# taichi-dev/taichi-nerfs

Hardware: AMD Instinct MI355X
Metric: training rays/sec (higher is better)
Workload: dtype f32-table+f16-mlp

## Files before the change

### taichi-nerfs_amd/csrc/march.hip

```cpp
#include "ngp_device.h"
#include "march_common.h"
#include <stdlib.h>

namespace ngp {

__global__ void __launch_bounds__(256) ray_aabb_kernel(const float* __restrict__ rays_o, const float* __restrict__ rays_d,
                                                        float scale, int n, float2* __restrict__ hits_t) {
    int r = blockIdx.x * blockDim.x + threadIdx.x;
    if (r >= n) return;
    float o[3], d_inv[3];
#pragma unroll
    for (int k = 0; k < 3; ++k) { o[k] = rays_o[3 * r + k]; d_inv[k] = 1.0f / rays_d[3 * r + k]; }
    hits_t[r] = ray_aabb_slab(o, d_inv, scale);
}

constexpr int MARCH_GROUP = 32;

template <bool CONST_DT, int G, bool CASC1>
__device__ __forceinline__ int march_rays_of_wave(const float* __restrict__ rays_o, const float* __restrict__ rays_d,
                                                  const float2* __restrict__ hits_t, const uint8_t* __restrict__ bits,
                                                  const float* __restrict__ noise, const MarchParams& p, int max_samples, int n_rays,
                                                  const uint32_t* __restrict__ coarse_s, bool use_coarse, float2* __restrict__ stage,
                                                  unsigned long long* __restrict__ chain, int first_ray, float o[3], float d[3]) {
    const int lane = threadIdx.x & 63;
    const int grp = lane / G, sub = lane % G;
    const int r = first_ray + grp;
    const bool has_ray = r < n_rays;
    const int rr = has_ray ? r : 0;
    float d_inv[3];
#pragma unroll
    for (int k = 0; k < 3; ++k) { o[k] = rays_o[3 * rr + k]; d[k] = rays_d[3 * rr + k]; d_inv[k] = 1.0f / d[k]; }
    float2 h;
    if (hits_t) h = hits_t[rr];
    else h = ray_aabb_slab(o, d_inv, p.scale);
    float t1 = h.x;
    const float t2 = h.y;
    const float dt_c = calc_dt(0.0f, p.esf, p.dt_min, p.dt_max);
    if (t1 >= 0.0f) t1 += calc_dt(t1, p.esf, p.dt_min, p.dt_max) * (p.rng ? rng_uniform(p.rng_seed, (unsigned int)rr) : noise[rr]);
    float t = t1;
    int n = 0;
    float t_target = -INFINITY;
    float2* row = stage + (size_t)rr * (size_t)max_samples;
    bool live = has_ray && (0.0f <= t) && (t < t2) && (n < max_samples);
    while (__any(live)) {
        float tu = t, t_last = t, tt = t;
        if (CONST_DT) {
#pragma unroll
            for (int k = 0; k < G; ++k) {
                tu = (k == sub) ? tt : tu;
                t_last = tt;
                tt += dt_c;
            }
        } else {
            for (int k = 0; k < G; ++k) {
                if (k == sub) tu = tt;
                t_last = tt;
                tt += calc_dt(tt, p.esf, p.dt_min, p.dt_max);
            }
        }
        const float t_next_batch = tt;
        const float dtu = CONST_DT ? dt_c : calc_dt(tu, p.esf, p.dt_min, p.dt_max);
        const float t_after = tu + dtu;
        CellProbe c;
        probe_cell<CASC1>(p, o, d, tu, dtu, c);
        bool occ = live;
        if (use_coarse && occ) { const uint32_t cb = c.idx >> 9; occ = (coarse_s[cb >> 5] >> (cb & 31u)) & 1u; }
        if (occ) occ = (bits[c.idx >> 3] >> (c.idx & 7u)) & 1u;
        const float targ = skip_target(p, d, d_inv, tu, c);
        const unsigned long long interesting = __ballot(live && (occ || targ > t_after));
        const unsigned long long gmask = (G == 64) ? ~0ull : (((1ull << (G & 63)) - 1ull) << ((grp * G) & 63));
        const bool need = (interesting & gmask) != 0ull;
        if (!need) {
            if (live) {
                if (!(t_last < t2)) live = false;
                if (!(t_target > t_last)) t_target = -INFINITY;
            }
        }
        if (interesting != 0ull) {
            const unsigned long long GM = (G == 64) ? ~0ull : ((1ull << (G & 63)) - 1ull);
            const int gbase = grp * G;
            const int gsh = gbase & 63;
            const bool act = live && need;
            const int nv = __popcll((__ballot(tu < t2) >> gsh) & GM);
            const int e0 = __popcll((__ballot(tu < t_target) >> gsh) & GM);
            const unsigned long long occm = (__ballot(occ) >> gsh) & GM;
            int c = 0;
#pragma unroll
            for (int s = G / 2; s >= 1; s >>= 1) {
                const float tv = __shfl(tu, gbase + c + s - 1);
                if (tv < targ) c += s;
            }
            if (__shfl(tu, gbase + G - 1) < targ) c = G;
            int j = occ ? sub + 1 : max(sub + 1, c);
            if (sub == 0) chain[grp] = (e0 < G) ? (1ull << e0) : 0ull;
            bool on_chain = sub == e0;
#pragma unroll
            for (int k = 1; k < G; k <<= 1) {
                wave_sync_lds();
                if (on_chain && j < G) atomicOr(&chain[grp], 1ull << j);
                wave_sync_lds();
                on_chain = (chain[grp] >> sub) & 1ull;
                if (2 * k < G) {
                    const int jj = __shfl(j, gbase + min(j, G - 1));
                    j = (j >= G) ? G : jj;
                }
            }
            const unsigned long long inside = (nv >= 64) ? ~0ull : ((1ull << nv) - 1ull);
            const unsigned long long X = act ? (chain[grp] & inside) : 0ull;
            const unsigned long long E = X & occm;
            const int cnt = __popcll(E), cap = max_samples - n;
            const int rank = __popcll(E & ((1ull << sub) - 1ull));
            if (((E >> sub) & 1ull) && rank < cap) row[n + rank] = make_float2(tu, dtu);
            const int last = X ? 63 - __clzll(X) : 0;
            const float targ_last = __shfl(targ, gbase + last);
            if (act) {
                if (X) t_target = ((occm >> last) & 1ull) ? -INFINITY : targ_last;
                const bool full = cnt >= cap;
                n = full ? max_samples : n + cnt;
                live = !full && nv == G;
            }
            wave_sync_lds();
        }
        t = t_next_batch;
    }
    return n;
}


template <bool CONST_DT, int G, bool CASC1>
__global__ void __launch_bounds__(64) march_count_kernel(const float* __restrict__ rays_o, const float* __restrict__ rays_d,
                                                         const float2* __restrict__ hits_t,
                                                         const uint8_t* __restrict__ bits, const float* __restrict__ noise,
                                                         MarchParams p, int max_samples, int n_rays,
                                                         const uint32_t* __restrict__ coarse ,
                                                         float2* __restrict__ stage, int32_t* __restrict__ counts) {
    constexpr int GROUPS = 64 / G;
    __shared__ unsigned long long chain[GROUPS];
    __shared__ uint32_t coarse_s[MARCH_MAX_COARSE_WORDS];
    const bool use_coarse = load_coarse(p, coarse, coarse_s);
    float o[3], d[3];
    const int n = march_rays_of_wave<CONST_DT, G, CASC1>(rays_o, rays_d, hits_t, bits, noise, p, max_samples, n_rays, coarse_s, use_coarse,
                                                         stage, chain, blockIdx.x * GROUPS, o, d);
    const int r = blockIdx.x * GROUPS + (int)threadIdx.x / G;
    if (r < n_rays && threadIdx.x % G == 0) counts[r] = n;
}

#ifdef NGP_MARCH_DIAG
__device__ unsigned long long ngp_march_dbg[4 * 8192];
#endif

template <bool CONST_DT, int G, bool CASC1, int WAVES>
__global__ void __launch_bounds__(64 * WAVES) march_fused_kernel(const float* __restrict__ rays_o, const float* __restrict__ rays_d,
                                                           const float2* __restrict__ hits_t, const uint8_t* __restrict__ bits,
                                                           const float* __restrict__ noise, MarchParams p, int max_samples, int n_rays,
                                                           const uint32_t* __restrict__ coarse, float2* __restrict__ stage,
                                                           int32_t* __restrict__ ctr, int32_t* __restrict__ rays_a,
                                                           int32_t* __restrict__ total, float* __restrict__ xyzs,
                                                           float* __restrict__ dirs, float* __restrict__ deltas, float* __restrict__ ts) {
    constexpr int GROUPS = 64 / G, RPB = WAVES * GROUPS;
    static_assert(RPB <= 64, "wave 0 scans the block's ray counts with one wave scan");
    __shared__ unsigned long long chain[WAVES][GROUPS];
    __shared__ uint32_t coarse_s[MARCH_MAX_COARSE_WORDS];
    __shared__ int s_off[RPB];
    const bool use_coarse = load_coarse(p, coarse, coarse_s);
    const int wv = threadIdx.x >> 6, lane = threadIdx.x & 63, grp = lane / G, sub = lane % G;
    const int first = blockIdx.x * RPB + wv * GROUPS, r = first + grp;
    float o[3], d[3];
#ifdef NGP_MARCH_DIAG
    const unsigned long long t_w0 = wall_clock64();
#endif
    const int n = march_rays_of_wave<CONST_DT, G, CASC1>(rays_o, rays_d, hits_t, bits, noise, p, max_samples, n_rays, coarse_s, use_coarse,
                                                         stage, chain[wv], first, o, d);
#ifdef NGP_MARCH_DIAG
    if (lane == 0 && blockIdx.x * WAVES + wv < 8192) {
        unsigned long long* q = ngp_march_dbg + 4 * (blockIdx.x * WAVES + wv);
        q[0] = t_w0; q[1] = wall_clock64(); q[3] = (unsigned long long)n;
    }
#endif
    const bool has_ray = r < n_rays;
    if (sub == 0) s_off[wv * GROUPS + grp] = has_ray ? n : 0;
    __threadfence_block();
    __syncthreads();
    if (wv == 0) {
        const int c = lane < RPB ? s_off[lane] : 0;
        const int inc = wave_scan_add_i(c, lane);
        int base = 0;
        if (lane == NGP_WAVE - 1) base = atomicAdd(&ctr[0], inc);
        base = __shfl(base, NGP_WAVE - 1, NGP_WAVE);
        if (lane < RPB) s_off[lane] = base + inc - c;
    }
    __syncthreads();
    if (has_ray) {
        const int start = s_off[wv * GROUPS + grp];
        if (sub == 0) { rays_a[3 * r] = r; rays_a[3 * r + 1] = start; rays_a[3 * r + 2] = n; }
        const float2* row = stage + (size_t)r * (size_t)max_samples;
        for (int k = sub; k < n; k += G) {
            const float2 s = row[k];
            const size_t g = (size_t)start + k;
            if (p.capacity > 0 && (long long)g >= p.capacity) break;
#pragma unroll
            for (int a = 0; a < 3; ++a) {
                xyzs[3 * g + a] = o[a] + s.x * d[a];
                dirs[3 * g + a] = d[a];
            }
            ts[g] = s.x;
            deltas[g] = s.y;
        }
    }
#ifdef NGP_MARCH_DIAG
    if (lane == 0 && blockIdx.x * WAVES + wv < 8192) ngp_march_dbg[4 * (blockIdx.x * WAVES + wv) + 2] = wall_clock64();
#endif
    if (threadIdx.x == 0) {
        if (atomicAdd(&ctr[1], 1) == (int)gridDim.x - 1) {
            total[0] = atomicExch(&ctr[0], 0);
            atomicExch(&ctr[1], 0);
        }
    }
}

__global__ void __launch_bounds__(256) bitfield_coarsen_kernel(const uint4* __restrict__ bits16, int n_coarse,
                                                               uint32_t* __restrict__ coarse) {
    const int w = blockIdx.x * blockDim.x + threadIdx.x;
    bool any = false;
    if (w < n_coarse) {
#pragma unroll
        for (int k = 0; k < 4; ++k) { const uint4 v = bits16[4 * (size_t)w + k]; any |= (v.x | v.y | v.z | v.w) != 0u; }
    }
    const unsigned long long m = __ballot(any);
    const int lane = threadIdx.x & 63;
    if (lane == 0 && w < n_coarse) coarse[w >> 5] = (uint32_t)m;
    if (lane == 32 && w < n_coarse) coarse[w >> 5] = (uint32_t)(m >> 32);
}

__global__ void __launch_bounds__(1024) march_scan_kernel(const int32_t* __restrict__ counts, int n_rays,
                                                          int32_t* __restrict__ rays_a, int32_t* __restrict__ total) {
    __shared__ int wave_tot[16];
    const int tid = threadIdx.x, lane = tid & 63, wv = tid >> 6;
    const int per = (n_rays + 1023) >> 10;
    const int lo = min(tid * per, n_rays), hi = min(lo + per, n_rays);
    int sum = 0;
    for (int i = lo; i < hi; ++i) sum += counts[i];
    const int inc = wave_scan_add_i(sum, lane);
    if (lane == 63) wave_tot[wv] = inc;
    __syncthreads();
    int woff = 0;
#pragma unroll
    for (int w = 0; w < 16; ++w) woff += (w < wv) ? wave_tot[w] : 0;
    int run = woff + inc - sum;
    for (int i = lo; i < hi; ++i) {
        const int c = counts[i];
        rays_a[3 * i] = i; rays_a[3 * i + 1] = run; rays_a[3 * i + 2] = c;
        run += c;
    }
    if (tid == 1023) total[0] = woff + inc;
}

__global__ void __launch_bounds__(1024) live_compact_kernel(const int32_t* __restrict__ rays_a, const int32_t* __restrict__ vr_per_ray,
                                                            int n_rays, int32_t* __restrict__ live_off, int32_t* __restrict__ live_idx,
                                                            int32_t* __restrict__ live_total) {
    __shared__ int wave_tot[16];
    const int tid = threadIdx.x, lane = tid & 63, wv = tid >> 6;
    const int per = (n_rays + 1023) >> 10;
    const int lo = min(tid * per, n_rays), hi = min(lo + per, n_rays);
    int sum = 0;
    for (int i = lo; i < hi; ++i) sum += vr_per_ray[i];
    const int inc = wave_scan_add_i(sum, lane);
    if (lane == 63) wave_tot[wv] = inc;
    __syncthreads();
    int woff = 0;
#pragma unroll
    for (int w = 0; w < 16; ++w) woff += (w < wv) ? wave_tot[w] : 0;
    int run = woff + inc - sum;
    for (int i = lo; i < hi; ++i) { live_off[i] = run; run += vr_per_ray[i]; }
    if (blockIdx.x == 0 && tid == 1023) live_total[0] = woff + inc;
    __threadfence_block();
    __syncthreads();
    const int share = (n_rays + (int)gridDim.x - 1) / (int)gridDim.x;
    const int n0 = blockIdx.x * share, n1 = min(n0 + share, n_rays);
    for (int n = n0 + wv; n < n1; n += 16) {
        const int ray = rays_a[3 * n], start = rays_a[3 * n + 1];
        const int cnt = vr_per_ray[ray], base = live_off[ray];
        for (int k = lane; k < cnt; k += NGP_WAVE) live_idx[base + k] = start + k;
    }
}

__global__ void __launch_bounds__(256) march_write_kernel(const float* __restrict__ rays_o, const float* __restrict__ rays_d,
                                                          const int32_t* __restrict__ rays_a, const float2* __restrict__ stage,
                                                          int max_samples, int n_rays, float* __restrict__ xyzs,
                                                          float* __restrict__ dirs, float* __restrict__ deltas,
                                                          float* __restrict__ ts) {
    int r = blockIdx.x * (blockDim.x >> 6) + (threadIdx.x >> 6);
    if (r >= n_rays) return;
    const int lane = lane_id();
    const int start = rays_a[3 * r + 1], cnt = rays_a[3 * r + 2];
    if (cnt == 0) return;
    float o[3], d[3];
#pragma unroll
    for (int k = 0; k < 3; ++k) { o[k] = rays_o[3 * r + k]; d[k] = rays_d[3 * r + k]; }
    const float2* row = stage + (size_t)r * (size_t)max_samples;
    for (int k = lane; k < cnt; k += NGP_WAVE) {
        float2 s = row[k];
        size_t g = (size_t)start + k;
#pragma unroll
        for (int a = 0; a < 3; ++a) {
            xyzs[3 * g + a] = o[a] + s.x * d[a];
            dirs[3 * g + a] = d[a];
        }
        ts[g] = s.x;
        deltas[g] = s.y;
    }
}

__global__ void __launch_bounds__(64) march_test_kernel(const float* __restrict__ rays_o, const float* __restrict__ rays_d,
                                                        float* __restrict__ hits_t, const int64_t* __restrict__ alive,
                                                        const uint8_t* __restrict__ bits, MarchParams p, int max_samples,
                                                        int n_alive, int64_t* __restrict__ ray_indices,
                                                        uint8_t* __restrict__ valid_mask, float* __restrict__ deltas,
                                                        float* __restrict__ ts, int32_t* __restrict__ samples_counter) {
    int n = blockIdx.x * blockDim.x + threadIdx.x;
    if (n >= n_alive) return;
    const int64_t r = alive[n];
    float o[3], d[3], d_inv[3];
#pragma unroll
    for (int k = 0; k < 3; ++k) { o[k] = rays_o[3 * r + k]; d[k] = rays_d[3 * r + k]; d_inv[k] = 1.0f / d[k]; }
    float t = hits_t[2 * r];
    const float t2 = hits_t[2 * r + 1];
    int s = 0;
    const size_t base = (size_t)n * (size_t)max_samples;
    float t_target = -INFINITY;
    float t_resume = t;
    bool wrote = false;
    bool live = (0.0f < t) && (t < t2) && (s < max_samples);
    while (live) {
        float tb[ORBIT_BATCH], dtb[ORBIT_BATCH];
        uint8_t ob[ORBIT_BATCH];
        uint32_t ib[ORBIT_BATCH];
        float tt = t;
#pragma unroll
        for (int u = 0; u < ORBIT_BATCH; ++u) {
            float dt = calc_dt(tt, p.esf, p.dt_min, p.dt_max);
            CellProbe c;
            probe_cell<false>(p, o, d, tt, dt, c);
            tb[u] = tt; dtb[u] = dt; ib[u] = c.idx;
            ob[u] = bits[c.idx >> 3];
            tt += dt;
        }
#pragma unroll
        for (int u = 0; u < ORBIT_BATCH; ++u) {
            if (!live) break;
            float tu = tb[u];
            if (!(tu < t2)) { live = false; break; }
            if (tu < t_target) continue;
            if (ob[u] & (1u << (ib[u] & 7u))) {
                size_t i = base + s;
                ray_indices[i] = r; valid_mask[i] = 1; ts[i] = tu; deltas[i] = dtb[u];
                t_resume = tu + dtb[u]; wrote = true;
                s += 1;
                t_target = -INFINITY;
                if (s >= max_samples) live = false;
            } else {
                CellProbe c;
                probe_cell<false>(p, o, d, tu, dtb[u], c);
                t_target = skip_target(p, d, d_inv, tu, c);
            }
        }
        t = tt;
    }
    if (wrote) hits_t[2 * r] = t_resume;
    samples_counter[n] = s;
}

}

using namespace ngp;

extern "C" {

int ngp_ray_aabb(const float* rays_o, const float* rays_d, float scale, int n_rays, float* hits_t, void* stream) {
    if (n_rays <= 0) return 0;
    hipLaunchKernelGGL(ray_aabb_kernel, dim3((n_rays + 255) / 256), dim3(256), 0, (hipStream_t)stream, rays_o, rays_d, scale,
                       n_rays, (float2*)hits_t);
    NGP_LAUNCH_CHECK();
    return 0;
}

int ngp_bitfield_coarsen(const uint8_t* density_bitfield, int cascades, int grid_size, uint32_t* coarse, void* stream) {
    const long long cells = (long long)cascades * grid_size * grid_size * grid_size;
    if (cells <= 0 || cells % 512 != 0) return -1;
    const int n_coarse = (int)(cells / 512);
    if (n_coarse % 32 != 0) return -1;
    hipLaunchKernelGGL(bitfield_coarsen_kernel, dim3((n_coarse + 255) / 256), dim3(256), 0, (hipStream_t)stream,
                       (const uint4*)density_bitfield, n_coarse, coarse);
    NGP_LAUNCH_CHECK();
    return 0;
}

int ngp_march_train_count(const float* rays_o, const float* rays_d, const float* hits_t, const uint8_t* density_bitfield,
                          const float* noise, int cascades, int grid_size, float scale, float exp_step_factor,
                          int max_samples, int n_rays, float* stage, int32_t* counts, void* stream) {
    return ngp_march_train_count_ex(rays_o, rays_d, hits_t, density_bitfield, nullptr, noise, cascades, grid_size, scale,
                                    exp_step_factor, max_samples, n_rays, stage, counts, stream);
}

int ngp_march_train_count_ex(const float* rays_o, const float* rays_d, const float* hits_t, const uint8_t* density_bitfield,
                             const uint32_t* coarse, const float* noise, int cascades, int grid_size, float scale,
                             float exp_step_factor, int max_samples, int n_rays, float* stage, int32_t* counts, void* stream) {
    if (n_rays <= 0) return 0;
    MarchParams p = make_march_params(cascades, grid_size, scale, exp_step_factor);
    const char* ge = ngp_experiment("march_group");
    const int group = ge ? atoi(ge) : MARCH_GROUP;
    hipStream_t s = (hipStream_t)stream;
#define NGP_LAUNCH_MARCH(CD, GG, C1)                                                                                           \
    hipLaunchKernelGGL((march_count_kernel<CD, GG, C1>), dim3((n_rays + 64 / GG - 1) / (64 / GG)), dim3(64), 0, s, rays_o,     \
                       rays_d, (const float2*)hits_t, density_bitfield, noise, p, max_samples, n_rays, coarse, (float2*)stage, \
                       counts)
    const bool cd = exp_step_factor == 0.0f, c1 = cascades == 1;
    if (group == 64) {
        if (cd && c1) NGP_LAUNCH_MARCH(true, 64, true); else if (cd) NGP_LAUNCH_MARCH(true, 64, false);
        else if (c1) NGP_LAUNCH_MARCH(false, 64, true); else NGP_LAUNCH_MARCH(false, 64, false);
    } else if (group == 16) {
        if (cd && c1) NGP_LAUNCH_MARCH(true, 16, true); else if (cd) NGP_LAUNCH_MARCH(true, 16, false);
        else if (c1) NGP_LAUNCH_MARCH(false, 16, true); else NGP_LAUNCH_MARCH(false, 16, false);
    } else {
        if (cd && c1) NGP_LAUNCH_MARCH(true, 32, true); else if (cd) NGP_LAUNCH_MARCH(true, 32, false);
        else if (c1) NGP_LAUNCH_MARCH(false, 32, true); else NGP_LAUNCH_MARCH(false, 32, false);
    }
#undef NGP_LAUNCH_MARCH
    NGP_LAUNCH_CHECK();
    return 0;
}

static int march_train_fused(const float* rays_o, const float* rays_d, const float* hits_t, const uint8_t* density_bitfield,
                             const uint32_t* coarse, const float* noise, bool rng, unsigned long long seed, int cascades, int grid_size,
                             float scale, float exp_step_factor, int max_samples, int n_rays, float* stage, int32_t* ctr, int32_t* rays_a,
                             int32_t* total, float* xyzs, float* dirs, float* deltas, float* ts, void* stream, long long capacity = 0,
                             int block_waves = 16, int lds_pad = 0) {
    if (n_rays <= 0) return 0;
    if (!ctr || !rays_a || !total || (!rng && !noise) || capacity < 0) return -1;
    if ((block_waves != 16 && block_waves != 8 && block_waves != 4) || lds_pad < 0 || lds_pad > 150 * 1024) return -1;
    MarchParams p = make_march_params(cascades, grid_size, scale, exp_step_factor);
    p.rng = rng ? 1 : 0; p.rng_seed = seed; p.capacity = capacity;
    hipStream_t s = (hipStream_t)stream;
    const int rpb = block_waves * (64 / MARCH_GROUP);
#define NGP_LAUNCH_MARCH_W(CD, C1, W)                                                                                               \
    hipLaunchKernelGGL((march_fused_kernel<CD, MARCH_GROUP, C1, W>), dim3((n_rays + rpb - 1) / rpb), dim3(64 * W), (size_t)lds_pad, s,   \
                       rays_o, rays_d, (const float2*)hits_t, density_bitfield, noise, p, max_samples, n_rays, coarse, (float2*)stage,  \
                       ctr, rays_a, total, xyzs, dirs, deltas, ts)
#define NGP_LAUNCH_MARCH(CD, C1)                                                                                                    \
    do { if (block_waves == 16) NGP_LAUNCH_MARCH_W(CD, C1, 16); else if (block_waves == 8) NGP_LAUNCH_MARCH_W(CD, C1, 8);           \
         else NGP_LAUNCH_MARCH_W(CD, C1, 4); } while (0)
    const bool cd = exp_step_factor == 0.0f, c1 = cascades == 1;
    if (cd && c1) NGP_LAUNCH_MARCH(true, true); else if (cd) NGP_LAUNCH_MARCH(true, false);
    else if (c1) NGP_LAUNCH_MARCH(false, true); else NGP_LAUNCH_MARCH(false, false);
#undef NGP_LAUNCH_MARCH
#undef NGP_LAUNCH_MARCH_W
    NGP_LAUNCH_CHECK();
    return 0;
}

int ngp_march_train_fused(const float* rays_o, const float* rays_d, const float* hits_t, const uint8_t* density_bitfield,
                          const uint32_t* coarse, const float* noise, int cascades, int grid_size, float scale, float exp_step_factor,
                          int max_samples, int n_rays, float* stage, int32_t* ctr, int32_t* rays_a, int32_t* total, float* xyzs,
                          float* dirs, float* deltas, float* ts, void* stream) {
    return march_train_fused(rays_o, rays_d, hits_t, density_bitfield, coarse, noise, false, 0ull, cascades, grid_size, scale,
                             exp_step_factor, max_samples, n_rays, stage, ctr, rays_a, total, xyzs, dirs, deltas, ts, stream);
}

int ngp_march_train_fused_cap(const float* rays_o, const float* rays_d, const float* hits_t, const uint8_t* density_bitfield,
                              const uint32_t* coarse, const float* noise, int cascades, int grid_size, float scale,
                              float exp_step_factor, int max_samples, int n_rays, long long capacity, float* stage, int32_t* ctr,
                              int32_t* rays_a, int32_t* total, float* xyzs, float* dirs, float* deltas, float* ts, void* stream) {
    return march_train_fused(rays_o, rays_d, hits_t, density_bitfield, coarse, noise, false, 0ull, cascades, grid_size, scale,
                             exp_step_factor, max_samples, n_rays, stage, ctr, rays_a, total, xyzs, dirs, deltas, ts, stream, capacity);
}

int ngp_march_train_fused_rng(const float* rays_o, const float* rays_d, const float* hits_t, const uint8_t* density_bitfield,
                              const uint32_t* coarse, unsigned long long seed, int cascades, int grid_size, float scale,
                              float exp_step_factor, int max_samples, int n_rays, float* stage, int32_t* ctr, int32_t* rays_a,
                              int32_t* total, float* xyzs, float* dirs, float* deltas, float* ts, void* stream) {
    return march_train_fused(rays_o, rays_d, hits_t, density_bitfield, coarse, nullptr, true, seed, cascades, grid_size, scale,
                             exp_step_factor, max_samples, n_rays, stage, ctr, rays_a, total, xyzs, dirs, deltas, ts, stream);
}

int ngp_march_train_fused_shaped(const float* rays_o, const float* rays_d, const float* hits_t, const uint8_t* density_bitfield,
                                 const uint32_t* coarse, const float* noise, unsigned long long seed, int cascades, int grid_size,
                                 float scale, float exp_step_factor, int max_samples, int n_rays, int block_waves, int lds_pad_bytes,
                                 float* stage, int32_t* ctr, int32_t* rays_a, int32_t* total, float* xyzs, float* dirs, float* deltas,
                                 float* ts, void* stream) {
    return march_train_fused(rays_o, rays_d, hits_t, density_bitfield, coarse, noise, noise == nullptr, seed, cascades, grid_size, scale,
                             exp_step_factor, max_samples, n_rays, stage, ctr, rays_a, total, xyzs, dirs, deltas, ts, stream, 0,
                             block_waves, lds_pad_bytes);
}

__global__ void rng_uniform_kernel(unsigned long long seed, int n, float* __restrict__ out) {
    const int i = blockIdx.x * blockDim.x + threadIdx.x;
    if (i < n) out[i] = rng_uniform(seed, (unsigned int)i);
}

int ngp_rng_uniform(unsigned long long seed, int n, float* out, void* stream) {
    if (n <= 0) return 0;
    hipLaunchKernelGGL(rng_uniform_kernel, dim3((n + 255) / 256), dim3(256), 0, (hipStream_t)stream, seed, n, out);
    NGP_LAUNCH_CHECK();
    return 0;
}

#ifdef NGP_MARCH_DIAG
int ngp_march_debug_read(unsigned long long* host, int n_words) {
    return hipMemcpyFromSymbol(host, HIP_SYMBOL(ngp_march_dbg), sizeof(unsigned long long) * (size_t)n_words) == hipSuccess ? 0 : -1;
}
#endif

int ngp_march_train_scan(const int32_t* counts, int n_rays, int32_t* rays_a, int32_t* total, void* stream) {
    hipLaunchKernelGGL(march_scan_kernel, dim3(1), dim3(1024), 0, (hipStream_t)stream, counts, n_rays, rays_a, total);
    NGP_LAUNCH_CHECK();
    return 0;
}

int ngp_live_compact(const int32_t* rays_a, const int32_t* vr_per_ray, int n_rays, int32_t* live_off, int32_t* live_idx,
                     int32_t* live_total, void* stream) {
    if (n_rays <= 0) return 0;
    int blocks = (n_rays + 127) / 128;
    if (blocks > 64) blocks = 64;
    hipLaunchKernelGGL(live_compact_kernel, dim3(blocks), dim3(1024), 0, (hipStream_t)stream, rays_a, vr_per_ray, n_rays, live_off, live_idx,
                       live_total);
    NGP_LAUNCH_CHECK();
    return 0;
}

int ngp_march_train_write(const float* rays_o, const float* rays_d, const int32_t* rays_a, const float* stage,
                          int max_samples, int n_rays, float* xyzs, float* dirs, float* deltas, float* ts, void* stream) {
    if (n_rays <= 0) return 0;
    hipLaunchKernelGGL(march_write_kernel, dim3((n_rays + 3) / 4), dim3(256), 0, (hipStream_t)stream, rays_o, rays_d, rays_a,
                       (const float2*)stage, max_samples, n_rays, xyzs, dirs, deltas, ts);
    NGP_LAUNCH_CHECK();
    return 0;
}

int ngp_march_test(const float* rays_o, const float* rays_d, float* hits_t, const int64_t* alive_indices,
                   const uint8_t* density_bitfield, int cascades, int grid_size, float scale, float exp_step_factor,
                   int max_samples, int n_alive, int64_t* ray_indices, uint8_t* valid_mask, float* deltas, float* ts,
                   int32_t* samples_counter, void* stream) {
    if (n_alive <= 0) return 0;
    MarchParams p = make_march_params(cascades, grid_size, scale, exp_step_factor);
    hipLaunchKernelGGL(march_test_kernel, dim3((n_alive + 63) / 64), dim3(64), 0, (hipStream_t)stream, rays_o, rays_d, hits_t,
                       alive_indices, density_bitfield, p, max_samples, n_alive, ray_indices, valid_mask, deltas, ts,
                       samples_counter);
    NGP_LAUNCH_CHECK();
    return 0;
}

}
```

### taichi-nerfs_amd/csrc/march_common.h

```cpp
#pragma once
#include "ngp_device.h"

namespace ngp {

struct MarchParams {
    int cascades, grid_size;
    uint32_t grid_size3;
    float grid_size_f, grid_size_inv, grid_max;
    float scale, esf, dt_min, dt_max;
    float scale_inv, mb0, mb0_inv;
    unsigned long long rng_seed;
    int rng;
    long long capacity;
};

__host__ inline MarchParams make_march_params(int cascades, int grid_size, float scale, float esf) {
    MarchParams p;
    p.cascades = cascades;
    p.grid_size = grid_size;
    p.grid_size3 = (uint32_t)grid_size * (uint32_t)grid_size * (uint32_t)grid_size;
    p.grid_size_f = (float)grid_size;
    p.grid_size_inv = 1.0f / (float)grid_size;
    p.grid_max = (float)grid_size - 1.0f;
    p.rng_seed = 0ull; p.rng = 0; p.capacity = 0;
    p.scale = scale;
    p.esf = esf;
    p.dt_min = (float)(1.7320508075688772 / 1024);
    p.dt_max = (float)(1.7320508075688772 * 2) * scale / (float)grid_size;
    p.scale_inv = 1.0f / scale;
    p.mb0 = 0.5f < scale ? 0.5f : scale;
    p.mb0_inv = 1.0f / p.mb0;
    return p;
}

struct CellProbe {
    float xyz[3];
    float nxyz[3];
    float mip_bound;
    uint32_t idx;
};

template <bool CASC1>
__device__ __forceinline__ void probe_cell(const MarchParams& p, const float o[3], const float d[3], float t, float dt,
                                           CellProbe& c) {
#pragma unroll
    for (int k = 0; k < 3; ++k) c.xyz[k] = o[k] + t * d[k];
    float mip_bound_inv;
    int mip = 0;
    if (CASC1) {
        c.mip_bound = p.mb0;
        mip_bound_inv = p.mb0_inv;
    } else {
        float mx = fmaxf(fmaxf(fabsf(c.xyz[0]), fabsf(c.xyz[1])), fabsf(c.xyz[2]));
        int mip_pos = min(p.cascades - 1, max(0, frexp_bit(mx) + 1));
        int mip_dt = min(p.cascades - 1, max(0, frexp_bit(dt * p.grid_size_f)));
        mip = max(mip_pos, mip_dt);
        const float pw = ldexpf(1.0f, mip - 1);
        const bool use_pw = pw <= p.scale;
        c.mip_bound = use_pw ? pw : p.scale;
        mip_bound_inv = use_pw ? ldexpf(1.0f, 1 - mip) : p.scale_inv;
    }
#pragma unroll
    for (int k = 0; k < 3; ++k) {
        float v = 0.5f * (c.xyz[k] * mip_bound_inv + 1.0f) * p.grid_size_f;
        c.nxyz[k] = fminf(p.grid_max, fmaxf(0.0f, v));
    }
    c.idx = (uint32_t)mip * p.grid_size3 + morton3d((uint32_t)c.nxyz[0], (uint32_t)c.nxyz[1], (uint32_t)c.nxyz[2]);
}

__device__ __forceinline__ float skip_target(const MarchParams& p, const float d[3], const float d_inv[3], float t,
                                             const CellProbe& c) {
    float tmin = 0.0f;
#pragma unroll
    for (int k = 0; k < 3; ++k) {
        float v = (((c.nxyz[k] + 0.5f + 0.5f * fsign(d[k])) * p.grid_size_inv * 2.0f - 1.0f) * c.mip_bound - c.xyz[k]) * d_inv[k];
        tmin = k ? fminf(tmin, v) : v;
    }
    return t + fmaxf(0.0f, tmin);
}

__device__ __forceinline__ float2 ray_aabb_slab(const float o[3], const float d_inv[3], float scale) {
    const float half_size = (scale - (-scale)) / 2.0f;
    float a1 = 0.f, a2 = 0.f;
#pragma unroll
    for (int k = 0; k < 3; ++k) {
        const float t_min = (0.0f - half_size - o[k]) * d_inv[k], t_max = (0.0f + half_size - o[k]) * d_inv[k];
        const float lo = fminf(t_min, t_max), hi = fmaxf(t_min, t_max);
        a1 = k ? fmaxf(a1, lo) : lo;
        a2 = k ? fminf(a2, hi) : hi;
    }
    return (a2 > 0.0f) ? make_float2(fmaxf(a1, 0.01f), a2) : make_float2(-1.0f, -1.0f);
}

__device__ __forceinline__ void wave_sync_lds() {
    __builtin_amdgcn_fence(__ATOMIC_ACQ_REL, "wavefront");
    __builtin_amdgcn_wave_barrier();
}

constexpr int MARCH_MAX_COARSE_WORDS = 1024;
constexpr int ORBIT_BATCH = 8;

__device__ __forceinline__ bool load_coarse(const MarchParams& p, const uint32_t* __restrict__ coarse, uint32_t* __restrict__ coarse_s) {
    const int coarse_words = coarse ? (int)((p.grid_size3 >> 9) * (uint32_t)p.cascades + 31u) >> 5 : 0;
    const bool use_coarse = coarse != nullptr && coarse_words <= MARCH_MAX_COARSE_WORDS;
    if (use_coarse) {
        for (int k = threadIdx.x; k < coarse_words; k += blockDim.x) coarse_s[k] = coarse[k];
        __syncthreads();
    }
    return use_coarse;
}

}
```

Before: 17.76 million.

## Compute constant-dt march positions in closed form and skip chain when no skips

For constant step size, the per-lane sample position is computed directly from the float bit pattern as t plus sub times a fixed ulp increment, whenever repeated float addition provably stays within one binade with exact rounding. Otherwise it falls back to the serial accumulation loop. The occupancy ballot is split from the skip ballot so the LDS chain-propagation loop and its barriers run only when some lane can skip empty space. The cell byte load is also issued before skip_target so its latency overlaps that computation. A microbenchmark script compares two builds for bitwise-identical output.

```diff
diff --git a/profiles/microbench/march_closed_form_ab.py b/profiles/microbench/march_closed_form_ab.py
--- /dev/null
+++ b/profiles/microbench/march_closed_form_ab.py
@@ -0,0 +1,103 @@
+import argparse
+import ctypes
+import json
+import os
+import sys
+from types import SimpleNamespace
+
+ROOT = os.path.dirname(os.path.dirname(os.path.dirname(os.path.abspath(__file__))))
+sys.path.insert(0, ROOT)
+sys.path.insert(0, os.path.join(ROOT, "taichi-nerfs_amd"))
+import numpy as np
+import torch
+from ngp_hip import lib, ops, synthetic
+
+N, MS = 8192, 1024
+ROUNDS, REP = 10, 20
+
+
+def load_local(path):
+    L = ctypes.CDLL(path)
+    for name, argtypes in lib.SIGNATURES.items():
+        fn = getattr(L, name)
+        fn.argtypes = argtypes
+        fn.restype = lib.RESTYPES[name]
+    return L
+
+
+def main():
+    ap = argparse.ArgumentParser()
+    ap.add_argument("--other", default=None, help="libngp_hip.so of the build to compare with (same ABI)")
+    ap.add_argument("--solo", action="store_true")
+    ap.add_argument("--out", default=None)
+    a = ap.parse_args()
+    dev = torch.device("cuda:0")
+    bits = torch.from_numpy(np.load(os.path.join(ROOT, "tests", "golden", "lego_density_bitfield.npz"))["density_bitfield"]).to(dev)
+    o, d = synthetic.lego_rays(N, seed=23)
+    o, d = torch.from_numpy(o).to(dev), torch.from_numpy(d).to(dev)
+    noise = torch.from_numpy(np.random.default_rng(0).random(N, dtype=np.float32)).to(dev)
+    if a.solo:
+        lib.load()
+        for shape in (None, (4, 0)):
+            for _ in range(20):
+                r = ops.march_train_fused(o, d, None, bits, noise, 1, 0.5, 0.0, 128, MS, shape=shape)
+            torch.cuda.synchronize()
+        print("total samples", int(r[5]))
+        return
+    if not a.other:
+        ap.error("--other or --solo")
+    L = {"this": load_local(lib.LIB_PATH), "other": load_local(a.other)}
+    lib._lib = L["this"]
+    coarse = ops.coarse_bitfield(bits, 1, 128)
+    hits = ops.ray_aabb(o, d, 0.5)
+    f32 = dict(device=dev, dtype=torch.float32)
+
+    def bufs():
+        cap = N * MS
+        return SimpleNamespace(stage=torch.empty(cap, 2, **f32), rays_a=torch.empty(N, 3, device=dev, dtype=torch.int32),
+                               total=torch.zeros(1, device=dev, dtype=torch.int32), ctr=torch.zeros(2, device=dev, dtype=torch.int32),
+                               xyzs=torch.empty(cap, 3, **f32), dirs=torch.empty(cap, 3, **f32), deltas=torch.empty(cap, **f32),
+                               ts=torch.empty(cap, **f32), counts=torch.empty(N, device=dev, dtype=torch.int32))
+    M = {w: bufs() for w in L}
+
+    def run(w, shape=None, ray_order=False):
+        ops.launch_march_train(L[w], M[w], o, d, hits if ray_order else None, bits, coarse, noise, 0, 1, 128, 0.5, 0.0, MS,
+                               shape=shape, ray_order=ray_order)
+
+    def gathered(m):
+        ra = m.rays_a.cpu().numpy()
+        idx = np.concatenate([np.arange(s, s + c) for _, s, c in ra]).astype(np.int64)
+        return ra[:, [0, 2]], m.ts.cpu().numpy()[idx].view(np.uint32), m.xyzs.cpu().numpy()[idx].view(np.uint32)
+    for w in L:
+        run(w)
+    torch.cuda.synchronize()
+    for x, y in zip(gathered(M["this"]), gathered(M["other"])):
+        assert np.array_equal(x, y), "the two builds disagree"
+    total = int(M["this"].total)
+    print("identical per-ray output, total samples", total, flush=True)
+    res = {}
+    for name, shape, ro in (("fused16", None, False), ("shaped4", (4, 0), False), ("shaped8", (8, 0), False), ("count_chain", None, True)):
+        for w in L:
+            for _ in range(3):
+                run(w, shape, ro)
+        torch.cuda.synchronize()
+        t = {w: [] for w in L}
+        for r in range(ROUNDS):
+            for w in (("other", "this") if r % 2 == 0 else ("this", "other")):
+                e0, e1 = torch.cuda.Event(enable_timing=True), torch.cuda.Event(enable_timing=True)
+                e0.record()
+                for _ in range(REP):
+                    run(w, shape, ro)
+                e1.record()
+                e1.synchronize()
+                t[w].append(e0.elapsed_time(e1) * 1e3 / REP)
+        res[name] = {w: {"median_us": float(np.median(t[w])), "min_us": float(np.min(t[w])), "max_us": float(np.max(t[w]))} for w in t}
+        print(name, json.dumps(res[name]), flush=True)
+    if a.out:
+        with open(a.out, "w") as f:
+            json.dump({"what": "us per launch, back-to-back launches (%d per timing, %d interleaved rounds)" % (REP, ROUNDS),
+                       "total_samples": total, "cases": res}, f, indent=1)
+
+
+if __name__ == "__main__":
+    main()
diff --git a/taichi-nerfs_amd/csrc/march.hip b/taichi-nerfs_amd/csrc/march.hip
--- a/taichi-nerfs_amd/csrc/march.hip
+++ b/taichi-nerfs_amd/csrc/march.hip
@@ -45,11 +45,23 @@
     while (__any(live)) {
         float tu = t, t_last = t, tt = t;
         if (CONST_DT) {
-#pragma unroll
-            for (int k = 0; k < G; ++k) {
-                tu = (k == sub) ? tt : tu;
-                t_last = tt;
-                tt += dt_c;
+            uint32_t q = 0u;
+            const bool closed = orbit_step_ulps<G>(t, dt_c, q);
+            const uint32_t tb = __float_as_uint(t);
+            tu = __uint_as_float(tb + (uint32_t)sub * q);
+            t_last = __uint_as_float(tb + (uint32_t)(G - 1) * q);
+            tt = __uint_as_float(tb + (uint32_t)G * q);
+            if (!__all(closed || !live)) {
+                float wu = t, wl = t, wt = t;
+#pragma unroll
+                for (int k = 0; k < G; ++k) {
+                    wu = (k == sub) ? wt : wu;
+                    wl = wt;
+                    wt += dt_c;
+                }
+                tu = closed ? tu : wu;
+                t_last = closed ? t_last : wl;
+                tt = closed ? tt : wt;
             }
         } else {
             for (int k = 0; k < G; ++k) {
@@ -65,9 +77,13 @@
         probe_cell<CASC1>(p, o, d, tu, dtu, c);
         bool occ = live;
         if (use_coarse && occ) { const uint32_t cb = c.idx >> 9; occ = (coarse_s[cb >> 5] >> (cb & 31u)) & 1u; }
-        if (occ) occ = (bits[c.idx >> 3] >> (c.idx & 7u)) & 1u;
+        uint32_t cell_byte = 0u;
+        if (occ) cell_byte = bits[c.idx >> 3];
         const float targ = skip_target(p, d, d_inv, tu, c);
-        const unsigned long long interesting = __ballot(live && (occ || targ > t_after));
+        occ = (cell_byte >> (c.idx & 7u)) & 1u;
+        const unsigned long long occ_w = __ballot(occ);
+        const unsigned long long skip_w = __ballot(live && !occ && targ > t_after);
+        const unsigned long long interesting = occ_w | skip_w;
         const unsigned long long gmask = (G == 64) ? ~0ull : (((1ull << (G & 63)) - 1ull) << ((grp * G) & 63));
         const bool need = (interesting & gmask) != 0ull;
         if (!need) {
@@ -83,30 +99,35 @@
             const bool act = live && need;
             const int nv = __popcll((__ballot(tu < t2) >> gsh) & GM);
             const int e0 = __popcll((__ballot(tu < t_target) >> gsh) & GM);
-            const unsigned long long occm = (__ballot(occ) >> gsh) & GM;
-            int c = 0;
-#pragma unroll
-            for (int s = G / 2; s >= 1; s >>= 1) {
-                const float tv = __shfl(tu, gbase + c + s - 1);
-                if (tv < targ) c += s;
-            }
-            if (__shfl(tu, gbase + G - 1) < targ) c = G;
-            int j = occ ? sub + 1 : max(sub + 1, c);
-            if (sub == 0) chain[grp] = (e0 < G) ? (1ull << e0) : 0ull;
-            bool on_chain = sub == e0;
-#pragma unroll
-            for (int k = 1; k < G; k <<= 1) {
+            const unsigned long long occm = (occ_w >> gsh) & GM;
+            unsigned long long marked = (e0 < G) ? (GM & ~((1ull << (e0 & 63)) - 1ull)) : 0ull;
+            if (skip_w != 0ull) {
+                int c = 0;
+#pragma unroll
+                for (int s = G / 2; s >= 1; s >>= 1) {
+                    const float tv = __shfl(tu, gbase + c + s - 1);
+                    if (tv < targ) c += s;
+                }
+                if (__shfl(tu, gbase + G - 1) < targ) c = G;
+                int j = occ ? sub + 1 : max(sub + 1, c);
+                if (sub == 0) chain[grp] = (e0 < G) ? (1ull << e0) : 0ull;
+                bool on_chain = sub == e0;
+#pragma unroll
+                for (int k = 1; k < G; k <<= 1) {
+                    wave_sync_lds();
+                    if (on_chain && j < G) atomicOr(&chain[grp], 1ull << j);
+                    wave_sync_lds();
+                    on_chain = (chain[grp] >> sub) & 1ull;
+                    if (2 * k < G) {
+                        const int jj = __shfl(j, gbase + min(j, G - 1));
+                        j = (j >= G) ? G : jj;
+                    }
+                }
+                marked = chain[grp];
                 wave_sync_lds();
-                if (on_chain && j < G) atomicOr(&chain[grp], 1ull << j);
-                wave_sync_lds();
-                on_chain = (chain[grp] >> sub) & 1ull;
-                if (2 * k < G) {
-                    const int jj = __shfl(j, gbase + min(j, G - 1));
-                    j = (j >= G) ? G : jj;
-                }
             }
             const unsigned long long inside = (nv >= 64) ? ~0ull : ((1ull << nv) - 1ull);
-            const unsigned long long X = act ? (chain[grp] & inside) : 0ull;
+            const unsigned long long X = act ? (marked & inside) : 0ull;
             const unsigned long long E = X & occm;
             const int cnt = __popcll(E), cap = max_samples - n;
             const int rank = __popcll(E & ((1ull << sub) - 1ull));
@@ -119,7 +140,6 @@
                 n = full ? max_samples : n + cnt;
                 live = !full && nv == G;
             }
-            wave_sync_lds();
         }
         t = t_next_batch;
     }
diff --git a/taichi-nerfs_amd/csrc/march_common.h b/taichi-nerfs_amd/csrc/march_common.h
--- a/taichi-nerfs_amd/csrc/march_common.h
+++ b/taichi-nerfs_amd/csrc/march_common.h
@@ -79,6 +79,20 @@
     return t + fmaxf(0.0f, tmin);
 }
 
+template <int G>
+__host__ __device__ __forceinline__ bool orbit_step_ulps(float t, float dt, uint32_t& q) {
+    static_assert(G >= 1 && G <= 256, "G * q must fit 32 bits");
+    const uint32_t tb = __builtin_bit_cast(uint32_t, t), db = __builtin_bit_cast(uint32_t, dt);
+    const uint32_t et = tb >> 23, ed = db >> 23;
+    const uint32_t md = (db & 0x7fffffu) | 0x800000u;
+    const uint32_t s = et - ed;
+    const uint32_t sh = s < 24u ? s : 24u;
+    const uint32_t half = (1u << sh) >> 1, rem = md & ((1u << sh) - 1u);
+    q = (md + half) >> sh;
+    return (int)(tb - 0x00800000u < 0x7f000000u) & (int)(db - 0x00800000u < 0x7f000000u) & (int)(s <= 24u) & (int)(rem != half) &
+           (int)(q - 1u < 0x7fffffu) & (int)(((tb + (uint32_t)G * q) >> 23) == et);
+}
+
 __device__ __forceinline__ float2 ray_aabb_slab(const float o[3], const float d_inv[3], float scale) {
     const float half_size = (scale - (-scale)) / 2.0f;
     float a1 = 0.f, a2 = 0.f;
```

Result: no change. 17.74 million, median of 3 (-0.1%).
